# ShuoYangRobotics/Cerberus

Measured on NVIDIA H100. Metric: sliding-window solves/sec (10-frame x 150-feature windows), higher is better.
Workload: dtype f64

## Files before the change

### cerberus_b200/csrc/compat.h

```cpp
#pragma once
#include <math.h>
#include <stdint.h>
#if defined(CERB_CUSIM)
#include "cusim.h"
#else
#include <cuda_runtime.h>
#define CERB_HD __host__ __device__ __forceinline__
#define CERB_D __device__ __forceinline__
#define CERB_GLOBAL __global__
#define CERB_NOINLINE __device__ __noinline__
#define CERB_GRID_CONSTANT const __grid_constant__
#define CERB_DYN_SMEM(T, name)                                   \
    extern __shared__ __align__(16) unsigned char name##_raw[]; \
    T *name = reinterpret_cast<T *>(name##_raw)
#define CERB_LAUNCH(kernel, grid, block, smem, stream, ...) kernel<<<(grid), (block), (smem), (stream)>>>(__VA_ARGS__)
#define CERB_BAR_SYNC(id, nthreads) asm volatile("bar.sync %0, %1;" ::"r"(id), "r"(nthreads) : "memory")
#define CERB_CP_ASYNC8(dst_smem, src_global) asm volatile("cp.async.ca.shared.global [%0], [%1], 8;" ::"r"((unsigned)__cvta_generic_to_shared(dst_smem)), "l"(src_global) : "memory")
#define CERB_CP_ASYNC_WAIT() asm volatile("cp.async.commit_group;\n\tcp.async.wait_group 0;" ::: "memory")
#define CERB_SMEM_U32(p) ((unsigned)__cvta_generic_to_shared(p))
#define CERB_MBAR_INIT(bar) do { asm volatile("mbarrier.init.shared::cta.b64 [%0], 1;" ::"r"(CERB_SMEM_U32(bar))); asm volatile("fence.mbarrier_init.release.cluster;" ::: "memory"); } while (0)
#define CERB_BULK_G2S(dst_smem, src_global, bytes, bar) do {                                                                                        \
        asm volatile("fence.proxy.async.shared::cta;" ::: "memory");                                                                                 \
        asm volatile("mbarrier.arrive.expect_tx.shared::cta.b64 _, [%0], %1;" ::"r"(CERB_SMEM_U32(bar)), "r"((unsigned)(bytes)) : "memory");         \
        asm volatile("cp.async.bulk.shared::cluster.global.mbarrier::complete_tx::bytes [%0], [%1], %2, [%3];"                                      \
                     ::"r"(CERB_SMEM_U32(dst_smem)), "l"(src_global), "r"((unsigned)(bytes)), "r"(CERB_SMEM_U32(bar)) : "memory");                   \
    } while (0)
#define CERB_MBAR_WAIT(bar, parity) do {                                                                                                             \
        unsigned done_ = 0;                                                                                                                          \
        while (!done_) asm volatile("{ .reg .pred p; mbarrier.try_wait.parity.shared::cta.b64 p, [%1], %2; selp.u32 %0, 1, 0, p; }"                 \
                                    : "=r"(done_) : "r"(CERB_SMEM_U32(bar)), "r"((unsigned)(parity)) : "memory");                                    \
    } while (0)
#define CERB_ST_RELEASE_S32(p, v) asm volatile("st.release.cta.shared.s32 [%0], %1;" ::"r"(CERB_SMEM_U32(p)), "r"((int)(v)) : "memory")
#define CERB_LD_ACQUIRE_S32(p) ({ int v_; asm volatile("ld.acquire.cta.shared.s32 %0, [%1];" : "=r"(v_) : "r"(CERB_SMEM_U32(p)) : "memory"); v_; })
#define CERB_SPIN_PAUSE() __nanosleep(20)
#define CERB_BAR_ARRIVE(id, nthreads) asm volatile("bar.arrive %0, %1;" ::"r"(id), "r"(nthreads) : "memory")
#define CERB_DMMA(d0, d1, a, b, c0, c1) \
    asm volatile("mma.sync.aligned.m8n8k4.row.col.f64.f64.f64.f64 {%0,%1}, {%2}, {%3}, {%4,%5};" : "=d"(d0), "=d"(d1) : "d"(a), "d"(b), "d"(c0), "d"(c1))
#endif
```

### cerberus_b200/csrc/solve_kernel.cuh

```cuda
#pragma once
#include "eval_kernels.cuh"

namespace cerb {

#if defined(CERB_PHASE_TIMING) && !defined(CERB_CUSIM)
__device__ unsigned long long g_phase_cycles[48];
#define PH_DECL() long long ph_t = clock64()
#define PH_MARK_T(id, t) do { if ((threadIdx.x & 31) == 0) { const long long ph_n = clock64(); if (threadIdx.x == (t)) atomicAdd(&g_phase_cycles[id], (unsigned long long)(ph_n - ph_t)); ph_t = ph_n; } __syncwarp(); } while (0)
#define PH_MARK(id) PH_MARK_T(id, 0)
#define PH_ARG , long long &ph_t
#define PH_FWD , ph_t
#else
#define PH_DECL()
#define PH_MARK_T(id, t)
#define PH_MARK(id)
#define PH_ARG
#define PH_FWD
#endif

enum { CERB_WINDOW = 10, NX = 79, NYB = 13, NFR = 11, NY = 143, NR = 222, NRP = 224, HXX_SZ = 79 * 79, HXY_SZ = 79 * 143, X_TD = 78, SOLVE_THREADS = 256, FT = 64, TILE_LD = 33, NOBS_PLANES = 9 };
enum { HBLK = NYB * NYB, AD_SZ = NFR * HBLK, BO_SZ = (NFR - 1) * HBLK };
#ifndef CERB_SOLVE_MIN_BLOCKS
#define CERB_SOLVE_MIN_BLOCKS 1
#endif
// ... 263 lines not shown
            }
            double wjv[6] = {0, 0, 0, 0, 0, 0};
            double *t0 = T + tid, *t1 = T + 256 + tid;
            if (valid) {
                const d3 tic = ld3(x + ST_EX), tc = kind == PROJ_K1 ? tic : ld3(x + ST_EX + 7);
                const double *Rcp = kind == PROJ_K1 ? s.Rex : s.Rex + 9;
                const double tdv = x[ST_TD];
                const d3 pts_i = mk3(pix, piy, 1.0), vel_i = mk3(vix, viy, 0.0);
                const d3 pts_i_td = pts_i - (tdv - tdi) * vel_i;
                const double pjx_td = ov.px - (tdv - ov.td) * ov.vx, pjy_td = ov.py - (tdv - ov.td) * ov.vy;
                const double inv_l = lamf;
                const d3 p_ci = inv_l * pts_i_td;
                const d3 p_bi = mv33(ldm33(s.Rex), p_ci) + tic;
                d3 p_bj = p_bi;
                if (kind != PROJ_K3) p_bj = mTv33(ldm33(s.Rw + 9 * j), (mv33(ldm33(s.Rw + 9 * a), p_bi) + ld3(x + ST_POSE + 7 * a)) - ld3(x + ST_POSE + 7 * j));
                const d3 p_cj = mTv33(ldm33(Rcp), p_bj - tc);
                const double iz = 1.0 / p_cj.z;
                double r0 = P.sqrt_info * (p_cj.x * iz - pjx_td), r1 = P.sqrt_info * (p_cj.y * iz - pjy_td);
                double cf; const double hw = huber_weight(P.huber, r0 * r0 + r1 * r1, &cf);
                cost += cf;
                r0 *= hw; r1 *= hw;
                const double q = hw * P.sqrt_info * iz, c0 = -q * p_cj.x * iz, c1 = -q * p_cj.y * iz;
                const d3 e0 = mk3(q, 0.0, c0), e1 = mk3(0.0, q, c1);
#define VIS_U(M, u0, u1) const d3 u0 = mk3(q * (M)[0] + c0 * (M)[6], q * (M)[1] + c0 * (M)[7], q * (M)[2] + c0 * (M)[8]), u1 = mk3(q * (M)[3] + c1 * (M)[6], q * (M)[4] + c1 * (M)[7], q * (M)[5] + c1 * (M)[8])
#define VIS_PUT(col, a0, a1) do { t0[(col) * VT_LD] = (a0); t1[(col) * VT_LD] = (a1); } while (0)
#define VIS_PUT3(col, v0_, v1_) do { VIS_PUT(col, (v0_).x, (v1_).x); VIS_PUT((col) + 1, (v0_).y, (v1_).y); VIS_PUT((col) + 2, (v0_).z, (v1_).z); } while (0)
                const double *Tm = kind == PROJ_K3 ? s.lin + 540 : s.lin + 27 * (2 * (j - a - 1) + cam) + 18;
                VIS_U(Tm, uT0, uT1);
                const d3 ptl = kind == PROJ_K3 ? pts_i : pts_i_td;
                const double l0 = -inv_l * inv_l * dot3(uT0, ptl), l1 = -inv_l * inv_l * dot3(uT1, ptl);
                const double d0 = -inv_l * dot3(uT0, vel_i) + hw * P.sqrt_info * ov.vx, d1 = -inv_l * dot3(uT1, vel_i) + hw * P.sqrt_info * ov.vy;
                h += l0 * l0 + l1 * l1; gq += l0 * r0 + l1 * r1; wT += d0 * l0 + d1 * l1;
                VIS_PUT(6, d0, d1); VIS_PUT(7, r0, r1);
                const d3 uC0 = mk3(q * Rcp[0] + c0 * Rcp[2], q * Rcp[3] + c0 * Rcp[5], q * Rcp[6] + c0 * Rcp[8]);
                const d3 uC1 = mk3(q * Rcp[1] + c1 * Rcp[2], q * Rcp[4] + c1 * Rcp[5], q * Rcp[7] + c1 * Rcp[8]);
                const d3 er0 = cross3(e0, p_cj), er1 = cross3(e1, p_cj);
                const d3 et0 = cross3(p_ci, uT0), et1 = cross3(p_ci, uT1);
                d3 E0t0, E0t1, E0r0, E0r1, E1t0, E1t1, E1r0, E1r1;
                if (kind == PROJ_K3) {
                    for (int k = 0; k < 6; k++) { VIS_PUT(k, 0.0, 0.0); VIS_PUT(8 + k, 0.0, 0.0); }
                    E0t0 = uC0; E0t1 = uC1; E0r0 = et0; E0r1 = et1; E1t0 = -uC0; E1t1 = -uC1; E1r0 = er0; E1r1 = er1;
                } else {
                    const double *C = s.lin + 27 * (2 * (j - a - 1) + cam);
                    VIS_U(C, uA0, uA1);
                    VIS_U(C + 9, uR0, uR1);
                    const d3 ir0 = cross3(p_bi, uR0), ir1 = cross3(p_bi, uR1);
                    const d3 jr0 = cross3(uC0, p_bj), jr1 = cross3(uC1, p_bj);
                    VIS_PUT3(0, uA0, uA1); VIS_PUT3(3, ir0, ir1);
                    VIS_PUT3(8, -uA0, -uA1); VIS_PUT3(11, jr0, jr1);
                    wI[0] += uA0.x * l0 + uA1.x * l1; wI[1] += uA0.y * l0 + uA1.y * l1; wI[2] += uA0.z * l0 + uA1.z * l1;
                    wI[3] += ir0.x * l0 + ir1.x * l1; wI[4] += ir0.y * l0 + ir1.y * l1; wI[5] += ir0.z * l0 + ir1.z * l1;
                    wjv[0] = -(uA0.x * l0 + uA1.x * l1); wjv[1] = -(uA0.y * l0 + uA1.y * l1); wjv[2] = -(uA0.z * l0 + uA1.z * l1);
                    wjv[3] = jr0.x * l0 + jr1.x * l1; wjv[4] = jr0.y * l0 + jr1.y * l1; wjv[5] = jr0.z * l0 + jr1.z * l1;
                    if (kind == PROJ_K1) {
                        E0t0 = uR0 - uC0; E0t1 = uR1 - uC1; E0r0 = et0 + er0; E0r1 = et1 + er1;
                        E1t0 = mk3(0, 0, 0); E1t1 = E1t0; E1r0 = E1t0; E1r1 = E1t0;
                    } else {
                        E0t0 = uR0; E0t1 = uR1; E0r0 = et0; E0r1 = et1; E1t0 = -uC0; E1t1 = -uC1; E1r0 = er0; E1r1 = er1;
                    }
                }
                VIS_PUT3(14, E0t0, E0t1); VIS_PUT3(17, E0r0, E0r1); VIS_PUT3(20, E1t0, E1t1); VIS_PUT3(23, E1r0, E1r1);
                wE0[0] += E0t0.x * l0 + E0t1.x * l1; wE0[1] += E0t0.y * l0 + E0t1.y * l1; wE0[2] += E0t0.z * l0 + E0t1.z * l1;
                wE0[3] += E0r0.x * l0 + E0r1.x * l1; wE0[4] += E0r0.y * l0 + E0r1.y * l1; wE0[5] += E0r0.z * l0 + E0r1.z * l1;
                wE1[0] += E1t0.x * l0 + E1t1.x * l1; wE1[1] += E1t0.y * l0 + E1t1.y * l1; wE1[2] += E1t0.z * l0 + E1t1.z * l1;
                wE1[3] += E1r0.x * l0 + E1r1.x * l1; wE1[4] += E1r0.y * l0 + E1r1.y * l1; wE1[5] += E1r0.z * l0 + E1r1.z * l1;
#undef VIS_U
#undef VIS_PUT
#undef VIS_PUT3
            } else {
                for (int k = 0; k < VT_COLS; k++) { t0[k * VT_LD] = 0.0; t1[k * VT_LD] = 0.0; }
            }
            const bool wrow = valid && j != a;
            if (wrow && cam == 0) for (int k = 0; k < 6; k++) W[(size_t)(6 * j + k) * F + f] = wjv[k] * (prescale ? s.sc[6 * j + k] * slf : 1.0);
            __syncthreads();
            PH_MARK(21);
            double wprev[6] = {0, 0, 0, 0, 0, 0};
            if (wrow && cam == 1) for (int k = 0; k < 6; k++) wprev[k] = W[(size_t)(6 * j + k) * F + f];
            { const int jn = j + 2; ov.stereo = 0; if (ev && jn < a + nobs) obs_fetch(obs, stereo, mo, off + (jn - a), cam, ov); }
            {
                const int jw = j0 + (wid >> 2), hw = (wid >> 1) & 1, par = wid & 1;
                const bool k3 = (jw == a);
                const int nkt = (nc + 3) >> 2;
                const bool work = jw < NFR && par < nkt;
                double acc[10][2];
                for (int k = 0; k < 10; k++) { acc[k][0] = 0.0; acc[k][1] = 0.0; }
                if (work) {
                    const int rb0 = 256 * hw + 64 * (wid >> 2) + 4 * par;
                    if (!k3) {
                        double v0 = tq[0][rb0], v1 = tv[1] ? tq[1][rb0] : 0.0, v2 = tv[2] ? tq[2][rb0] : 0.0;
                        for (int ks = par; ks < nkt; ks += 2) {
                            const int rn = rb0 + 4 * (ks + 2 - par);
                            const bool more = ks + 2 < nkt;
                            const double n0 = more ? tq[0][rn] : 0.0, n1 = (more && tv[1]) ? tq[1][rn] : 0.0, n2 = (more && tv[2]) ? tq[2][rn] : 0.0;
                            CERB_DMMA(acc[0][0], acc[0][1], v0, v0, acc[0][0], acc[0][1]);
                            CERB_DMMA(acc[1][0], acc[1][1], v0, v1, acc[1][0], acc[1][1]);
                            CERB_DMMA(acc[2][0], acc[2][1], v0, v2, acc[2][0], acc[2][1]);
                            CERB_DMMA(acc[4][0], acc[4][1], v1, v1, acc[4][0], acc[4][1]);
                            CERB_DMMA(acc[5][0], acc[5][1], v1, v2, acc[5][0], acc[5][1]);
                            CERB_DMMA(acc[7][0], acc[7][1], v2, v2, acc[7][0], acc[7][1]);
                            v0 = n0; v1 = n1; v2 = n2;
                        }
                    }
                    {
                        const int rb1 = rb0 + 128;
                        double v0 = tq[0][rb1], v1 = (!k3 && tv[1]) ? tq[1][rb1] : 0.0, v2 = tv[2] ? tq[2][rb1] : 0.0, v3 = tv[3] ? tq[3][rb1] : 0.0;
                        for (int ks = par; ks < nkt; ks += 2) {
                            const int rn = rb1 + 4 * (ks + 2 - par);
                            const bool more = ks + 2 < nkt;
                            const double n0 = more ? tq[0][rn] : 0.0, n1 = (more && !k3 && tv[1]) ? tq[1][rn] : 0.0, n2 = (more && tv[2]) ? tq[2][rn] : 0.0, n3 = (more && tv[3]) ? tq[3][rn] : 0.0;
                            CERB_DMMA(acc[0][0], acc[0][1], v0, v0, acc[0][0], acc[0][1]);
                            CERB_DMMA(acc[2][0], acc[2][1], v0, v2, acc[2][0], acc[2][1]);
                            CERB_DMMA(acc[3][0], acc[3][1], v0, v3, acc[3][0], acc[3][1]);
                            CERB_DMMA(acc[7][0], acc[7][1], v2, v2, acc[7][0], acc[7][1]);
                            CERB_DMMA(acc[8][0], acc[8][1], v2, v3, acc[8][0], acc[8][1]);
                            CERB_DMMA(acc[9][0], acc[9][1], v3, v3, acc[9][0], acc[9][1]);
                            if (!k3) {
                                CERB_DMMA(acc[1][0], acc[1][1], v0, v1, acc[1][0], acc[1][1]);
                                CERB_DMMA(acc[4][0], acc[4][1], v1, v1, acc[4][0], acc[4][1]);
                                CERB_DMMA(acc[5][0], acc[5][1], v1, v2, acc[5][0], acc[5][1]);
                                CERB_DMMA(acc[6][0], acc[6][1], v1, v3, acc[6][0], acc[6][1]);
                            }
                            v0 = n0; v1 = n1; v2 = n2; v3 = n3;
                        }
                    }
                    PH_MARK(28);
                    const int o = (lane >> 2) * 8 + 2 * (lane & 3);
                    pp[0 * 64 + o] += acc[0][0]; pp[0 * 64 + o + 1] += acc[0][1];
                    pp[1 * 64 + o] += acc[2][0]; pp[1 * 64 + o + 1] += acc[2][1];
                    pp[2 * 64 + o] += acc[3][0]; pp[2 * 64 + o + 1] += acc[3][1];
                    pp[3 * 64 + o] += acc[7][0]; pp[3 * 64 + o + 1] += acc[7][1];
                    pp[4 * 64 + o] += acc[8][0]; pp[4 * 64 + o + 1] += acc[8][1];
                    pp[5 * 64 + o] += acc[9][0]; pp[5 * 64 + o + 1] += acc[9][1];
                }
                {
                    const int o = wid * VJ_SZ + (lane >> 2) * 8 + 2 * (lane & 3);
                    jp[o] = acc[1][0]; jp[o + 1] = acc[1][1];
                    jp[64 + o] = acc[4][0]; jp[64 + o + 1] = acc[4][1];
                    jp[128 + o] = acc[5][0]; jp[128 + o + 1] = acc[5][1];
                    jp[192 + o] = acc[6][0]; jp[192 + o + 1] = acc[6][1];
                }
            }
            if (wrow && cam == 1) for (int k = 0; k < 6; k++) W[(size_t)(6 * j + k) * F + f] = wprev[k] + wjv[k] * (prescale ? s.sc[6 * j + k] * slf : 1.0);
            PH_MARK(29);
            __syncthreads();
            PH_MARK(22);
            if (jbase >= 0) {
                _Pragma("unroll")
                for (int fj = 0; fj < 2; fj++) {
                    const int jf = j0 + fj;
                    if (jf >= NFR || jf == a) continue;
                    const double *q = jp + (4 * fj) * VJ_SZ + tid;
                    smem_base[jbase + jca * a + jcj * jf] += ((q[0] + q[VJ_SZ]) + q[2 * VJ_SZ]) + q[3 * VJ_SZ];
                }
            }
            PH_MARK(23);
        }
        __syncthreads();
        {
            double *ex = T;
            ex[0 * 256 + tid] = h; ex[1 * 256 + tid] = gq; ex[2 * 256 + tid] = wT;
            for (int k = 0; k < 6; k++) { ex[(3 + k) * 256 + tid] = wI[k]; ex[(9 + k) * 256 + tid] = wE0[k]; ex[(15 + k) * 256 + tid] = wE1[k]; }
        }
        __syncthreads();
        for (int e = tid; e < VP_SZ; e += SOLVE_THREADS) {
            double v = 0.0;
            for (int wq = 0; wq < 8; wq++) v += ((wq < 5) ? s.Ju + 8 * VJ_SZ + VP_SZ * wq : s.tile + VT_SZ + VP_SZ * (wq - 5))[e];
            const int blk = e >> 6, ra = (e >> 3) & 7, rb = e & 7;
            const int ga = blk < 3 ? 0 : (blk < 5 ? 2 : 3), gb = blk == 0 ? 0 : (blk == 1 || blk == 3 ? 2 : 3);
            vis_scatter(s, ga, gb, ra, rb, a, a, v);
        }
        if (tid < 64 && ev) {
            const double *ex = T;
            double q[21];
            for (int k = 0; k < 21; k++) q[k] = ((ex[k * 256 + tid] + ex[k * 256 + 64 + tid]) + ex[k * 256 + 128 + tid]) + ex[k * 256 + 192 + tid];
            hh[f] = q[0] * slf * slf; gl[f] = q[1] * slf;
            W[(size_t)X_TD * F + f] = q[2] * (prescale ? s.sc[X_TD] * slf : 1.0);
            for (int k = 0; k < 6; k++) {
                W[(size_t)(6 * a + k) * F + f] = q[3 + k] * (prescale ? s.sc[6 * a + k] * slf : 1.0);
                W[(size_t)(66 + k) * F + f] = q[9 + k] * (prescale ? s.sc[66 + k] * slf : 1.0);
                W[(size_t)(72 + k) * F + f] = q[15 + k] * (prescale ? s.sc[72 + k] * slf : 1.0);
            }
        }
        __syncthreads();
        PH_MARK(24);
    }
    return cost;
}

CERB_D void imu_lin_all(const SolveParams &P, Smem &s, int w, const double *x, bool want_jac, int tid) {
    if (tid < CERB_WINDOW) {
        const double *pre = P.pre + ((size_t)w * CERB_WINDOW + tid) * PRE_STRIDE;
        IMULegLin *L = reinterpret_cast<IMULegLin *>(s.lin + 96 * tid);
        imu_leg_linearize(pre, x + ST_POSE + 7 * tid, x + ST_SB + 9 * tid, x + ST_LB + 4 * tid, x + ST_POSE + 7 * (tid + 1),
                          x + ST_SB + 9 * (tid + 1), x + ST_LB + 4 * (tid + 1), P.G, want_jac, L);
    }
    __syncthreads();
}

CERB_D double prior_residual(const SolveParams &P, Smem &s, int w, const double *x, int tid) {
    const int *meta = P.prior_meta + (size_t)w * PRIOR_META_STRIDE;
    if (!meta[0]) return 0.0;
    const int n = meta[1], nb = meta[2];
    const double *J = P.prior_J + (size_t)w * PRIOR_LD * PRIOR_LD, *r0 = P.prior_r + (size_t)w * PRIOR_LD, *x0 = P.prior_x0 + (size_t)w * 16 * 9;
    if (tid < nb) {
        const int kind = meta[4 + 3 * tid], index = meta[5 + 3 * tid], col = meta[6 + 3 * tid];
        prior_block_dx(kind, x + prior_block_state_offset(kind, index), x0 + 9 * tid, s.pdx + col);
    }
    __syncthreads();
    int parts = SOLVE_THREADS / n; if (parts > 4) parts = 4; if (parts < 1) parts = 1;
    const int kc = (n + parts - 1) / parts;
    double *part = s.red;
    for (int e = tid; e < parts * n; e += SOLVE_THREADS) {
        const int p = e / n, i = e % n;
        const int k1 = (p + 1) * kc < n ? (p + 1) * kc : n;
        double t = 0.0;
        for (int k = p * kc; k < k1; k++) t += J[(size_t)k * n + i] * s.pdx[k];
        part[p * PRIOR_LD + i] = t;
    }
    __syncthreads();
    double cost = 0.0;
    for (int i = tid; i < n; i += SOLVE_THREADS) {
        double t = r0[i];
// ... 194 lines not shown
    for (int k = tid; k < NR; k += SOLVE_THREADS) s.g[k] += gp[k];
    __syncthreads();
    PH_MARK(27);
    return cost;
}

CERB_D void apply_plus(const Smem &s, const double *delta, const double *lam, const double *dlam, double *lamc, int nF, bool ex_open, bool td_open, int tid) {
    if (tid < 11) pose_plus(s.xs + ST_POSE + 7 * tid, delta + 6 * tid, s.xc + ST_POSE + 7 * tid);
    else if (tid < 13) {
        const int e = tid - 11;
        if (ex_open) pose_plus(s.xs + ST_EX + 7 * e, delta + 66 + 6 * e, s.xc + ST_EX + 7 * e);
        else for (int k = 0; k < 7; k++) s.xc[ST_EX + 7 * e + k] = s.xs[ST_EX + 7 * e + k];
    }
    for (int k = tid; k < 99; k += SOLVE_THREADS) { const int f = k / 9, c = k % 9; s.xc[ST_SB + k] = s.xs[ST_SB + k] + delta[NX + NYB * f + c]; }
    for (int k = tid; k < 44; k += SOLVE_THREADS) { const int f = k / 4, c = k % 4; s.xc[ST_LB + k] = s.xs[ST_LB + k] + delta[NX + NYB * f + 9 + c]; }
    if (tid == 0) s.xc[ST_TD] = td_open ? s.xs[ST_TD] + delta[X_TD] : s.xs[ST_TD];
    for (int f = tid; f < nF; f += SOLVE_THREADS) lamc[f] = lam[f] + dlam[f];
    __syncthreads();
}

CERB_D double ambient_sq(const double *a, const double *b, const double *la, const double *lb, int nF, bool ex_open, bool lb_open, bool td_open, int tid) {
    double t = 0.0;
    for (int k = tid; k < ST_SIZE; k += SOLVE_THREADS) {
        if (k >= ST_LB && k < ST_EX && !lb_open) continue;
        if (k >= ST_EX && k < ST_TD && !ex_open) continue;
        if (k == ST_TD && !td_open) continue;
        const double v = b ? a[k] - b[k] : a[k];
        t += v * v;
    }
    for (int f = tid; f < nF; f += SOLVE_THREADS) { const double v = lb ? la[f] - lb[f] : la[f]; t += v * v; }
    return t;
}

template <int W> struct TTPlan;
#define CERB_TT_PLAN(W, NR_, NB_, ...) template <> struct TTPlan<W> { static constexpr int nr = NR_, nb = NB_; static CERB_HD int tab(int i) { constexpr int t[] = {__VA_ARGS__}; return t[i]; } };
CERB_TT_PLAN(0, 4, 7, 0, 1, 2, 3, 0, 0, 0,   0, 0, 1, 0, 1, 0, 1,   0, 1, 1, 2, 2, 3, 3)
CERB_TT_PLAN(1, 4, 7, 2, 3, 4, 5, 0, 0, 0,   0, 0, 1, 0, 1, 0, 1,   0, 1, 1, 2, 2, 3, 3)
CERB_TT_PLAN(2, 4, 7, 4, 5, 6, 7, 0, 0, 0,   0, 0, 1, 0, 1, 0, 1,   0, 1, 1, 2, 2, 3, 3)
CERB_TT_PLAN(3, 4, 7, 6, 7, 8, 9, 0, 0, 0,   0, 0, 1, 0, 1, 0, 1,   0, 1, 1, 2, 2, 3, 3)
CERB_TT_PLAN(4, 6, 7, 8, 9, 0, 1, 4, 5, 0,   0, 0, 1, 2, 3, 2, 3,   0, 1, 1, 4, 4, 5, 5)
CERB_TT_PLAN(5, 6, 7, 0, 1, 6, 7, 8, 9, 0,   0, 0, 0, 0, 1, 1, 1,   2, 3, 4, 5, 2, 3, 4)
CERB_TT_PLAN(6, 7, 7, 1, 9, 2, 6, 7, 8, 3,   0, 2, 2, 2, 2, 6, 6,   1, 3, 4, 5, 1, 3, 4)
CERB_TT_PLAN(7, 5, 6, 3, 4, 5, 8, 9, 0, 0,   0, 0, 1, 1, 2, 2, 0,   3, 4, 3, 4, 3, 4, 0)
template <int W> CERB_D void ttt_warp(Smem &s, int lane) {
    typedef TTPlan<W> PL;
    const double *pr[7];
    _Pragma("unroll")
    for (int u = 0; u < 7; u++) {
        const int r = 8 * PL::tab(u < PL::nr ? u : 0) + (lane >> 2);
        pr[u] = (r < NX ? s.Hxy + r * NY : s.yv + NX) + (lane & 3);
    }
    double acc[7][2], fv[7];
    _Pragma("unroll")
    for (int k = 0; k < 7; k++) { acc[k][0] = 0.0; acc[k][1] = 0.0; }
    _Pragma("unroll")
    for (int u = 0; u < 7; u++) fv[u] = (u < PL::nr) ? pr[u][0] : 0.0;
    for (int q0 = 0; q0 < NY; q0 += 4) {
        const int qn = q0 + 4;
        const bool take = qn < NY && qn + (lane & 3) < NY;
        double fn[7];
        _Pragma("unroll")
        for (int u = 0; u < 7; u++) fn[u] = (u < PL::nr && take) ? pr[u][qn] : 0.0;
        _Pragma("unroll")
        for (int k = 0; k < 7; k++) if (k < PL::nb) CERB_DMMA(acc[k][0], acc[k][1], fv[PL::tab(7 + k)], fv[PL::tab(14 + k)], acc[k][0], acc[k][1]);
        _Pragma("unroll")
        for (int u = 0; u < 7; u++) fv[u] = fn[u];
    }
    _Pragma("unroll")
    for (int k = 0; k < 7; k++) {
        if (k >= PL::nb) continue;
        const int ba = PL::tab(PL::tab(7 + k)), bb = PL::tab(PL::tab(14 + k));
        const int a = 8 * ba + (lane >> 2);
        for (int e = 0; e < 2; e++) {
            const int b = 8 * bb + 2 * (lane & 3) + e;
            if (a > b || a >= NX || b > NX) continue;
            if (b == NX) s.yv[a] -= acc[k][e];
            else s.Hxx[b * NX + a] -= acc[k][e];
        }
    }
}

template <int W> struct SCPlan;
#define CERB_SC_PLAN(W, NR_, NB_, ...) template <> struct SCPlan<W> { static constexpr int nr = NR_, nb = NB_; static CERB_HD int tab(int i) { constexpr int t[] = {__VA_ARGS__}; return t[i]; } };
CERB_SC_PLAN(0, 8, 8, 0, 1, 2, 3, 4, 5, 6, 7, 0,   0, 0, 0, 0, 0, 0, 0, 0,   0, 1, 2, 3, 4, 5, 6, 7)
CERB_SC_PLAN(1, 9, 8, 0, 8, 9, 1, 2, 3, 4, 5, 6,   0, 0, 3, 3, 3, 3, 3, 3,   1, 2, 3, 4, 5, 6, 7, 8)
CERB_SC_PLAN(2, 9, 8, 1, 7, 8, 9, 2, 3, 4, 5, 6,   0, 0, 0, 4, 4, 4, 4, 4,   1, 2, 3, 4, 5, 6, 7, 8)
CERB_SC_PLAN(3, 8, 8, 2, 7, 8, 9, 3, 4, 5, 6, 0,   0, 0, 0, 4, 4, 4, 4, 4,   1, 2, 3, 4, 5, 6, 7, 1)
CERB_SC_PLAN(4, 7, 8, 3, 8, 9, 4, 5, 6, 7, 0, 0,   0, 0, 3, 3, 3, 3, 3, 3,   1, 2, 3, 4, 5, 6, 1, 2)
CERB_SC_PLAN(5, 5, 8, 5, 6, 7, 8, 9, 0, 0, 0, 0,   0, 0, 0, 0, 0, 1, 1, 1,   0, 1, 2, 3, 4, 1, 2, 3)
CERB_SC_PLAN(6, 4, 7, 6, 7, 8, 9, 0, 0, 0, 0, 0,   0, 1, 1, 1, 2, 2, 3, 0,   3, 1, 2, 3, 2, 3, 3, 0)
enum { SC_LDW = 36 };
template <int W> CERB_D void schur_tile(const double *tw, double (&acc)[8][2], int lane) {
    typedef SCPlan<W> PL;
    const double *pr[9];
    _Pragma("unroll")
    for (int u = 0; u < 9; u++) pr[u] = tw + (8 * PL::tab(u < PL::nr ? u : 0) + (lane >> 2)) * SC_LDW + (lane & 3);
    double fv[9];
    _Pragma("unroll")
    for (int u = 0; u < 9; u++) fv[u] = (u < PL::nr) ? pr[u][0] : 0.0;
    _Pragma("unroll")
    for (int ks = 0; ks < 8; ks++) {
        double fn[9];
        _Pragma("unroll")
        for (int u = 0; u < 9; u++) fn[u] = (u < PL::nr && ks < 7) ? pr[u][4 * (ks + 1)] : 0.0;
        _Pragma("unroll")
        for (int k = 0; k < 8; k++) if (k < PL::nb) CERB_DMMA(acc[k][0], acc[k][1], fv[PL::tab(9 + k)], fv[PL::tab(17 + k)], acc[k][0], acc[k][1]);
        _Pragma("unroll")
        for (int u = 0; u < 9; u++) fv[u] = fn[u];
    }
}
template <int W> CERB_D void schur_scatter(Smem &s, const double (&acc)[8][2], int lane) {
    typedef SCPlan<W> PL;
    _Pragma("unroll")
    for (int k = 0; k < 8; k++) {
        if (k >= PL::nb) continue;
        const int a = 8 * PL::tab(PL::tab(9 + k)) + (lane >> 2);
        for (int e = 0; e < 2; e++) {
            const int b = 8 * PL::tab(PL::tab(17 + k)) + 2 * (lane & 3) + e;
            if (a > b || a >= NX || b > NX) continue;
            if (b == NX) s.yv[a] -= acc[k][e];
            else { s.Hxx[b * NX + a] -= acc[k][e]; if (a != b) s.Hxx[a * NX + b] -= acc[k][e]; }
        }
    }
}

CERB_D bool build_prior_image(const SolveParams &P, Smem &s, int w, double *pimg, int tid) {
    const int *pmeta = P.prior_meta + (size_t)w * PRIOR_META_STRIDE;
    const bool has_prior = pmeta[0] != 0;
    if (has_prior) {
        const int n = pmeta[1], nb = pmeta[2];
        for (int k = tid; k < PIMG_SZ; k += SOLVE_THREADS) pimg[k] = 0.0;
        if (tid < nb) {
            const int kind = pmeta[4 + 3 * tid], index = pmeta[5 + 3 * tid], col = pmeta[6 + 3 * tid];
            const int local = (kind == 0 || kind == 3) ? 6 : prior_block_size(kind);
            for (int k = 0; k < local; k++) {
                int d;
                if (kind == 0) d = 6 * index + k;
                else if (kind == 3) d = 66 + 6 * index + k;
                else if (kind == 1) d = -(1 + NYB * index + k);
                else if (kind == 2) d = -(1 + NYB * index + 9 + k);
                else d = X_TD;
                s.ti[TI_PRIOR_MAP + col + k] = d;
            }
        }
        __syncthreads();
        Smem si = s; si.Hxx = pimg; si.Hxy = pimg + PIMG_HXY; si.Ad = pimg + PIMG_HXY + HXY_SZ; si.Bo = pimg + PIMG_HXY + HXY_SZ + AD_SZ;
        const double *Hp = P.prior_Hp + (size_t)w * PRIOR_LD * PRIOR_LD;
        for (int idx = tid; idx < n * n; idx += SOLVE_THREADS) {
            const int a = idx / n, b = idx % n;
            if (b < a) continue;
            scatter_H(si, s.ti[TI_PRIOR_MAP + a], s.ti[TI_PRIOR_MAP + b], Hp[a * PRIOR_LD + b]);
        }
    }
    return has_prior;
}

CERB_D void build_imu_plan(const Smem &s, const double *smem_base, int *plan, int tid) {
    if (tid >= 32) return;
    int q = 0;
    for (int mi = 0; mi < 5; mi++)
        for (int ni = mi; ni < 5; ni++, q++)
            for (int e = 0; e < 2; e++) {
                const int la = 8 * mi + (tid >> 2), lb = 8 * ni + 2 * (tid & 3) + e;
                int px = (int)(s.idg - smem_base) + tid, py = 256 << 12;
                if (la <= lb && lb <= 38 && la != 38) {
                    double *p0[2], *p1[2];
                    for (int i = 0; i < 2; i++) {
                        const int da = imu_col_dest(i, la);
                        if (lb == 38) { p0[i] = da >= 0 ? s.g + da : s.g + NX + (-da - 1); p1[i] = nullptr; }
                        else scatter_addr(s, da, imu_col_dest(i, lb), &p0[i], &p1[i]);
                    }
                    px = (int)(p0[0] - smem_base);
                    py = (int)(p0[1] - p0[0]) | (((p1[0] ? (int)(p1[0] - p0[0]) : 0) + 256) << 12);
                }
                plan[(2 * (q * 2 + e)) * 32 + tid] = px; plan[(2 * (q * 2 + e) + 1) * 32 + tid] = py;
            }
}
CERB_D void build_chunks(const int *fstart, Smem &s, int *chunks, int n_end) {
    int n = 0, c0 = 0;
    while (c0 < n_end) {
        chunks[1 + n] = c0;
        const int a = fstart[c0];
        int e = c0 + 1;
        while (e < n_end && e < c0 + 64 && fstart[e] == a) e++;
        if (n < TI_CACHED_CHUNKS) { s.ti[TI_CHUNK_CACHE + 2 * n] = c0; s.ti[TI_CHUNK_CACHE + 2 * n + 1] = ((e - c0) << 8) | a; }
        n++; c0 = e;
    }
    chunks[1 + n] = n_end; chunks[0] = n; s.ti[TI_NCHUNKS] = n;
}
struct Win { int w, nF; bool ex_open, lb_open, td_open, has_prior, bulk_ok; double *lam; CtaWs ws; };
struct PriorCopy { unsigned par0, par1; bool hxx_prefetched; };
CERB_D void linearize(const SolveParams &P, Smem &s, const Win &c, PriorCopy &pc, const double *xl, const double *laml, bool first, int tid PH_ARG) {
    const int F = c.ws.F, nF = c.nF;
    double *sca = s.sca, *W = c.ws.W, *hh = c.ws.hh, *gl = c.ws.gl, *sl = c.ws.sl, *pimg = c.ws.pimg;
    if (!c.has_prior) { for (int k = tid; k < HXX_SZ; k += SOLVE_THREADS) s.Hxx[k] = 0.0; }
    else if (c.bulk_ok) {
        if (!pc.hxx_prefetched) { __syncthreads(); if (tid == 0) CERB_BULK_G2S(s.Hxx, pimg, PIMG_HXY * 8, &s.mbar[0]); }
        CERB_MBAR_WAIT(&s.mbar[0], pc.par0); pc.par0 ^= 1;
    } else { if (!pc.hxx_prefetched) copy_g2s_async(s.Hxx, pimg, HXX_SZ, tid); CERB_CP_ASYNC_WAIT(); }
    pc.hxx_prefetched = false;
    for (int k = tid; k < NRP; k += SOLVE_THREADS) s.g[k] = 0.0;
    load_geometry(xl, s, tid);
    double part[2];
    PH_MARK(0);
// ... 58 lines not shown
    if (tid == 0) {
        if (iteration >= P.max_iters) { sca[S_DONE] = 1; sca[S_TERM] = 1; }
        else if (sca[S_GMAX] <= P.gtol) { sca[S_DONE] = 1; sca[S_TERM] = 0; }
        else if (sca[S_RADIUS] <= P.min_radius) { sca[S_DONE] = 1; sca[S_TERM] = 0; }
        else if (!(sca[S_XCOST] == sca[S_XCOST]) || fabs(sca[S_XCOST]) > 1e300) { sca[S_DONE] = 1; sca[S_TERM] = 2; }
    }
    __syncthreads();
    return sca[S_DONE] != 0.0;
}
CERB_D void dogleg_diagonal(Smem &s, const Win &c, int tid PH_ARG) {
    const int nF = c.nF;
    double *sca = s.sca, *Dl = c.ws.Dl, *ghl = c.ws.ghl, *stl = c.ws.stl;
    for (int k = tid; k < NR; k += SOLVE_THREADS) {
        const double d = (k < NX) ? s.Hxx[k * NX + k] : s.Ad[((k - NX) / NYB) * HBLK + ((k - NX) % NYB) * (NYB + 1)];
        const double D = sqrt(fmin(fmax(d, 1e-6), 1e32));
        s.D[k] = D; s.gh[k] = s.g[k] / D; s.stp[k] = s.gh[k] / D;
    }
    for (int f = tid; f < nF; f += SOLVE_THREADS) { const double D = sqrt(fmin(fmax(c.ws.hh[f], 1e-6), 1e32)); Dl[f] = D; ghl[f] = c.ws.gl[f] / D; stl[f] = ghl[f] / D; }
    __syncthreads();
    double part[2] = {0.0, 0.0};
    for (int k = tid; k < AD_SZ; k += SOLVE_THREADS) { const int f = k / HBLK, a = (k % HBLK) / NYB, b = k % NYB; part[0] += s.stp[NX + NYB * f + a] * s.Ad[k] * s.stp[NX + NYB * f + b]; }
    for (int k = tid; k < BO_SZ; k += SOLVE_THREADS) { const int f = k / HBLK, a = (k % HBLK) / NYB, b = k % NYB; part[0] += 2.0 * s.stp[NX + NYB * f + a] * s.Bo[k] * s.stp[NX + NYB * (f + 1) + b]; }
    for (int f = tid; f < nF; f += SOLVE_THREADS) part[1] += ghl[f] * ghl[f];
    for (int k = tid; k < NR; k += SOLVE_THREADS) part[1] += s.gh[k] * s.gh[k];
    double tot[2];
    block_sum<2>(part, s.red, tot, tid);
    if (tid == 0) { sca[S_GNORM2] = tot[1]; sca[S_VHV] = tot[0]; sca[S_OK] = 1; }
    PH_MARK(4);
}
CERB_D void chain_cholesky(Smem &s, int *chain_done, int lane PH_ARG) {
    const bool act = lane < NYB;
    const int r = act ? lane : 0;
    double m[NYB];
    _Pragma("unroll")
    for (int c = 0; c < NYB; c++) m[c] = 0.0;
    _Pragma("unroll 1")
    for (int f = 0; f < NFR; f++) {
        double *A = s.Ad + f * HBLK;
        double a[NYB], invd[NYB], myinv = 1.0;
        _Pragma("unroll")
        for (int c = 0; c < NYB; c++) a[c] = A[r * NYB + c];
        if (f > 0) {
            const double *Mp = s.Bo + (f - 1) * HBLK;
            _Pragma("unroll")
            for (int c = 0; c < NYB; c++) { double t = 0.0; _Pragma("unroll") for (int q = 0; q < NYB; q++) t += m[q] * Mp[c * NYB + q]; a[c] -= t; }
        }
        _Pragma("unroll")
        for (int j = 0; j < NYB; j++) {
            double d = __shfl_sync(0xffffffffu, a[j], j);
            if (!(d > 0.0)) { if (lane == 0) s.sca[S_OK] = 0; d = 1.0; }
            const double inv = rsqrt(d);
            invd[j] = inv;
            if (lane == j) myinv = inv;
            const double l = (lane == j) ? d * inv : a[j] * inv;
            a[j] = l;
            double *colb = s.chain_col + 16 * (j & 1);
            if (act) colb[lane] = l;
            __syncwarp();
            _Pragma("unroll")
            for (int k = j + 1; k < NYB; k++) a[k] -= l * colb[k];
        }
        if (act) { _Pragma("unroll") for (int c = 0; c < NYB; c++) if (c <= r) A[r * NYB + c] = a[c]; s.idg[NYB * f + r] = myinv; }
        __syncwarp();
        if (f < NFR - 1) {
            double *B = s.Bo + f * HBLK;
            double t[NYB];
            _Pragma("unroll")
            for (int c = 0; c < NYB; c++) t[c] = B[c * NYB + r];
            _Pragma("unroll")
            for (int c = 0; c < NYB; c++) {
                m[c] = t[c] * invd[c];
                _Pragma("unroll")
                for (int c2 = c + 1; c2 < NYB; c2++) t[c2] -= m[c] * A[c2 * NYB + c];
            }
            __syncwarp();
            if (act) { _Pragma("unroll") for (int c = 0; c < NYB; c++) B[r * NYB + c] = m[c]; }
            __syncwarp();
        }
        __threadfence_block(); __syncwarp();
        if (lane == 0) CERB_ST_RELEASE_S32(chain_done, f + 1);
    }
    PH_MARK(6);
}
CERB_D void schur_tile_w(int wq, const double *tw, double (&acc)[8][2], int lane) {
    switch (wq) { case 0: schur_tile<0>(tw, acc, lane); break; case 1: schur_tile<1>(tw, acc, lane); break; case 2: schur_tile<2>(tw, acc, lane); break;
                  case 3: schur_tile<3>(tw, acc, lane); break; case 4: schur_tile<4>(tw, acc, lane); break; case 5: schur_tile<5>(tw, acc, lane); break;
                  default: schur_tile<6>(tw, acc, lane); break; }
}
CERB_D void schur_scatter_w(int wq, Smem &s, const double (&acc)[8][2], int lane) {
    switch (wq) { case 0: schur_scatter<0>(s, acc, lane); break; case 1: schur_scatter<1>(s, acc, lane); break; case 2: schur_scatter<2>(s, acc, lane); break;
                  case 3: schur_scatter<3>(s, acc, lane); break; case 4: schur_scatter<4>(s, acc, lane); break; case 5: schur_scatter<5>(s, acc, lane); break;
                  default: schur_scatter<6>(s, acc, lane); break; }
}
CERB_D void ttt_warp_w(int wq, Smem &s, int lane) {
    switch (wq) { case 0: ttt_warp<0>(s, lane); break; case 1: ttt_warp<1>(s, lane); break; case 2: ttt_warp<2>(s, lane); break; case 3: ttt_warp<3>(s, lane); break;
                  case 4: ttt_warp<4>(s, lane); break; case 5: ttt_warp<5>(s, lane); break; case 6: ttt_warp<6>(s, lane); break; default: ttt_warp<7>(s, lane); break; }
}
CERB_D void lambda_schur(Smem &s, const Win &c, double mu, int tid PH_ARG) {
    const int F = c.ws.F, nF = c.nF;
    const double *W = c.ws.W, *hh = c.ws.hh, *gl = c.ws.gl, *Dl = c.ws.Dl, *stl = c.ws.stl;
    const int t2 = tid - 32, n2 = SOLVE_THREADS - 32;
    const int wq = (tid >> 5) - 1, lane = tid & 31;
    const int LDW = SC_LDW;
    double *tw = s.Ju;
    double *sinv = nF <= 1024 ? s.wj : c.ws.sinv;
    {
        const double *v = s.stp;
        double pv = 0.0;
        for (int k = t2; k < NX * NX; k += n2) pv += v[k / NX] * s.Hxx[k] * v[k % NX];
        for (int k = t2; k < NX * NY; k += n2) pv += 2.0 * v[k / NY] * s.Hxy[k] * v[NX + k % NY];
        for (int f = t2; f < nF; f += n2) {
            double wv = 0.0;
            for (int a = 0; a < NX; a++) wv += W[(size_t)a * F + f] * v[a];
            pv += 2.0 * stl[f] * wv + hh[f] * stl[f] * stl[f];
        }
        for (int o = 16; o > 0; o >>= 1) pv += __shfl_sync(0xffffffffu, pv, (lane + o) & 31);
        if (lane == 0) s.lin[wq] = pv;
        CERB_BAR_SYNC(1, n2);
        for (int k = t2; k < NX; k += n2) s.Hxx[k * NX + k] += mu * s.D[k] * s.D[k];
    }
    PH_MARK_T(19, 32);
    for (int f = t2; f < nF; f += n2) sinv[f] = rsqrt(hh[f] + mu * Dl[f] * Dl[f]);
    double acc[8][2];
    _Pragma("unroll")
    for (int k = 0; k < 8; k++) { acc[k][0] = 0.0; acc[k][1] = 0.0; }
    CERB_BAR_SYNC(1, n2);
    double buf[12];
    auto fetch = [&](int f0) {
        const int nf = (nF - f0) < 32 ? (nF - f0) : 32;
        _Pragma("unroll")
        for (int u = 0; u < 12; u++) {
            const int e = t2 + u * n2, a = e >> 5, f = e & 31;
            buf[u] = (e < 80 * 32 && f < nf) ? (a < NX ? W[(size_t)a * F + f0 + f] : (a == NX ? gl[f0 + f] : 0.0)) : 0.0;
        }
    };
    fetch(0);
    PH_MARK_T(37, 32);
    for (int f0 = 0; f0 < nF; f0 += 32) {
        const int nf = (nF - f0) < 32 ? (nF - f0) : 32;
        _Pragma("unroll")
        for (int u = 0; u < 12; u++) {
            const int e = t2 + u * n2, a = e >> 5, f = e & 31;
            if (e < 80 * 32) tw[a * LDW + f] = (f < nf) ? buf[u] * sinv[f0 + f] : 0.0;
        }
        CERB_BAR_SYNC(1, n2);
        PH_MARK_T(38, 32);
        if (f0 + 32 < nF) fetch(f0 + 32);
        schur_tile_w(wq, tw, acc, lane);
        CERB_BAR_SYNC(1, n2);
        PH_MARK_T(39, 32);
    }
    schur_scatter_w(wq, s, acc, lane);
    PH_MARK_T(7, 32);
}
CERB_D void forward_subst(Smem &s, const int *chain_done, int t2) {
    if (t2 <= NX) {
        double *row = (t2 < NX) ? s.Hxy + t2 * NY : s.yv + NX;
        double tp[NYB];
        _Pragma("unroll")
        for (int k = 0; k < NYB; k++) tp[k] = 0.0;
        _Pragma("unroll 1")
        for (int f = 0; f < NFR; f++) {
            while (CERB_LD_ACQUIRE_S32(chain_done) <= f) { CERB_SPIN_PAUSE(); }
            __threadfence_block();
            const double *L = s.Ad + f * HBLK, *idg = s.idg + NYB * f;
            double *t = row + NYB * f;
            double tc[NYB];
            _Pragma("unroll")
            for (int r = 0; r < NYB; r++) tc[r] = t[r];
            if (f > 0) {
                const double *M = s.Bo + (f - 1) * HBLK;
                _Pragma("unroll")
                for (int r = 0; r < NYB; r++) { double acc = 0.0; _Pragma("unroll") for (int q = 0; q < NYB; q++) acc += M[r * NYB + q] * tp[q]; tc[r] -= acc; }
            }
            _Pragma("unroll")
            for (int c = 0; c < NYB; c++) {
                tc[c] *= idg[c];
                _Pragma("unroll")
                for (int r = c + 1; r < NYB; r++) tc[r] -= L[r * NYB + c] * tc[c];
            }
            _Pragma("unroll")
            for (int r = 0; r < NYB; r++) { t[r] = tc[r]; tp[r] = tc[r]; }
        }
    }
}
CERB_D void panel_cholesky(Smem &s, int tid) {
    const int wq = tid >> 5, lane = tid & 31;
    auto factor_diag = [&](int c0, int nb, double *Lkk) {
        const bool act = lane < nb;
        const int r = act ? lane : 0;
        double a[8];
        _Pragma("unroll")
        for (int c = 0; c < 8; c++) a[c] = (c < nb && c <= r) ? s.Hxx[(c0 + r) * NX + c0 + c] : 0.0;
        double myinv = 1.0;
        _Pragma("unroll")
        for (int j = 0; j < 8; j++) {
            double d = __shfl_sync(0xffffffffu, a[j], j);
            if (j < nb && !(d > 0.0)) { if (lane == 0) s.sca[S_OK] = 0; }
            if (!(d > 0.0)) d = 1.0;
            const double inv = rsqrt(d);
            if (lane == j) myinv = inv;
            const double l = (lane == j) ? d * inv : a[j] * inv;
            a[j] = l;
            _Pragma("unroll")
            for (int k = j + 1; k < 8; k++) { const double lk = __shfl_sync(0xffffffffu, l, k); a[k] -= l * lk; }
        }
        if (act) {
            _Pragma("unroll")
// ... 483 lines not shown
```

Measured before the change: 29250.

## Pair FP64 8x8x4 DMMAs into m16n8k4 instructions in visibility and Schur tiles

Replaces pairs of m8n8k4 FP64 mma.sync ops sharing a B operand with single m16n8k4 instructions, in both the visibility-block accumulation and the Schur complement tile kernel. The Schur tiling plan tables are rewritten so each warp issues fewer, larger MMAs, and the scatter is updated for the new accumulator layout, including transposed indexing for some blocks. This cuts MMA instruction count and issue overhead. It also redistributes work across warps and relies on index mapping that is easy to get wrong.

```diff
diff --git a/cerberus_b200/csrc/compat.h b/cerberus_b200/csrc/compat.h
--- a/cerberus_b200/csrc/compat.h
+++ b/cerberus_b200/csrc/compat.h
@@ -3,6 +3,7 @@
 #include <stdint.h>
 #if defined(CERB_CUSIM)
 #include "cusim.h"
+#define CERB_DMMA_16x8x4(d0, d1, d2, d3, a0, a1, b) do { CERB_DMMA(d0, d1, a0, b, d0, d1); CERB_DMMA(d2, d3, a1, b, d2, d3); } while (0)
 #else
 #include <cuda_runtime.h>
 #define CERB_HD __host__ __device__ __forceinline__
@@ -36,4 +37,7 @@
 #define CERB_BAR_ARRIVE(id, nthreads) asm volatile("bar.arrive %0, %1;" ::"r"(id), "r"(nthreads) : "memory")
 #define CERB_DMMA(d0, d1, a, b, c0, c1) \
     asm volatile("mma.sync.aligned.m8n8k4.row.col.f64.f64.f64.f64 {%0,%1}, {%2}, {%3}, {%4,%5};" : "=d"(d0), "=d"(d1) : "d"(a), "d"(b), "d"(c0), "d"(c1))
+#define CERB_DMMA_16x8x4(d0, d1, d2, d3, a0, a1, b)                                                                                   \
+    asm volatile("mma.sync.aligned.m16n8k4.row.col.f64.f64.f64.f64 {%0,%1,%2,%3}, {%4,%5}, {%6}, {%0,%1,%2,%3};"                    \
+                 : "+d"(d0), "+d"(d1), "+d"(d2), "+d"(d3) : "d"(a0), "d"(a1), "d"(b))
 #endif
diff --git a/cerberus_b200/csrc/solve_kernel.cuh b/cerberus_b200/csrc/solve_kernel.cuh
--- a/cerberus_b200/csrc/solve_kernel.cuh
+++ b/cerberus_b200/csrc/solve_kernel.cuh
@@ -369,8 +369,9 @@
                 const bool k3 = (jw == a);
                 const int nkt = (nc + 3) >> 2;
                 const bool work = jw < NFR && par < nkt;
-                double acc[10][2];
-                for (int k = 0; k < 10; k++) { acc[k][0] = 0.0; acc[k][1] = 0.0; }
+                double acc[5][4];
+                for (int k = 0; k < 5; k++) { acc[k][0] = 0.0; acc[k][1] = 0.0; acc[k][2] = 0.0; acc[k][3] = 0.0; }
+#define VIS_Q(q, ga, gb, gc) CERB_DMMA_16x8x4(acc[q][0], acc[q][1], acc[q][2], acc[q][3], ga, gb, gc)
                 if (work) {
                     const int rb0 = 256 * hw + 64 * (wid >> 2) + 4 * par;
                     if (!k3) {
@@ -379,12 +380,7 @@
                             const int rn = rb0 + 4 * (ks + 2 - par);
                             const bool more = ks + 2 < nkt;
                             const double n0 = more ? tq[0][rn] : 0.0, n1 = (more && tv[1]) ? tq[1][rn] : 0.0, n2 = (more && tv[2]) ? tq[2][rn] : 0.0;
-                            CERB_DMMA(acc[0][0], acc[0][1], v0, v0, acc[0][0], acc[0][1]);
-                            CERB_DMMA(acc[1][0], acc[1][1], v0, v1, acc[1][0], acc[1][1]);
-                            CERB_DMMA(acc[2][0], acc[2][1], v0, v2, acc[2][0], acc[2][1]);
-                            CERB_DMMA(acc[4][0], acc[4][1], v1, v1, acc[4][0], acc[4][1]);
-                            CERB_DMMA(acc[5][0], acc[5][1], v1, v2, acc[5][0], acc[5][1]);
-                            CERB_DMMA(acc[7][0], acc[7][1], v2, v2, acc[7][0], acc[7][1]);
+                            VIS_Q(0, v0, v2, v0); VIS_Q(1, v1, v0, v1); VIS_Q(2, v2, v1, v2);
                             v0 = n0; v1 = n1; v2 = n2;
                         }
                     }
@@ -395,36 +391,27 @@
                             const int rn = rb1 + 4 * (ks + 2 - par);
                             const bool more = ks + 2 < nkt;
                             const double n0 = more ? tq[0][rn] : 0.0, n1 = (more && !k3 && tv[1]) ? tq[1][rn] : 0.0, n2 = (more && tv[2]) ? tq[2][rn] : 0.0, n3 = (more && tv[3]) ? tq[3][rn] : 0.0;
-                            CERB_DMMA(acc[0][0], acc[0][1], v0, v0, acc[0][0], acc[0][1]);
-                            CERB_DMMA(acc[2][0], acc[2][1], v0, v2, acc[2][0], acc[2][1]);
-                            CERB_DMMA(acc[3][0], acc[3][1], v0, v3, acc[3][0], acc[3][1]);
-                            CERB_DMMA(acc[7][0], acc[7][1], v2, v2, acc[7][0], acc[7][1]);
-                            CERB_DMMA(acc[8][0], acc[8][1], v2, v3, acc[8][0], acc[8][1]);
-                            CERB_DMMA(acc[9][0], acc[9][1], v3, v3, acc[9][0], acc[9][1]);
-                            if (!k3) {
-                                CERB_DMMA(acc[1][0], acc[1][1], v0, v1, acc[1][0], acc[1][1]);
-                                CERB_DMMA(acc[4][0], acc[4][1], v1, v1, acc[4][0], acc[4][1]);
-                                CERB_DMMA(acc[5][0], acc[5][1], v1, v2, acc[5][0], acc[5][1]);
-                                CERB_DMMA(acc[6][0], acc[6][1], v1, v3, acc[6][0], acc[6][1]);
-                            }
+                            VIS_Q(0, v0, v2, v0); VIS_Q(2, v2, v1, v2); VIS_Q(3, v0, v2, v3); VIS_Q(4, v3, v1, v3);
+                            if (!k3) VIS_Q(1, v1, v0, v1);
                             v0 = n0; v1 = n1; v2 = n2; v3 = n3;
                         }
                     }
                     PH_MARK(28);
-                    const int o = (lane >> 2) * 8 + 2 * (lane & 3);
+                    const int o = (lane >> 2) * 8 + 2 * (lane & 3), ot = 2 * (lane & 3) * 8 + (lane >> 2);
                     pp[0 * 64 + o] += acc[0][0]; pp[0 * 64 + o + 1] += acc[0][1];
-                    pp[1 * 64 + o] += acc[2][0]; pp[1 * 64 + o + 1] += acc[2][1];
+                    pp[1 * 64 + ot] += acc[0][2]; pp[1 * 64 + ot + 8] += acc[0][3];
                     pp[2 * 64 + o] += acc[3][0]; pp[2 * 64 + o + 1] += acc[3][1];
-                    pp[3 * 64 + o] += acc[7][0]; pp[3 * 64 + o + 1] += acc[7][1];
-                    pp[4 * 64 + o] += acc[8][0]; pp[4 * 64 + o + 1] += acc[8][1];
-                    pp[5 * 64 + o] += acc[9][0]; pp[5 * 64 + o + 1] += acc[9][1];
+                    pp[3 * 64 + o] += acc[2][0]; pp[3 * 64 + o + 1] += acc[2][1];
+                    pp[4 * 64 + o] += acc[3][2]; pp[4 * 64 + o + 1] += acc[3][3];
+                    pp[5 * 64 + o] += acc[4][0]; pp[5 * 64 + o + 1] += acc[4][1];
                 }
+#undef VIS_Q
                 {
                     const int o = wid * VJ_SZ + (lane >> 2) * 8 + 2 * (lane & 3);
-                    jp[o] = acc[1][0]; jp[o + 1] = acc[1][1];
-                    jp[64 + o] = acc[4][0]; jp[64 + o + 1] = acc[4][1];
-                    jp[128 + o] = acc[5][0]; jp[128 + o + 1] = acc[5][1];
-                    jp[192 + o] = acc[6][0]; jp[192 + o + 1] = acc[6][1];
+                    jp[o] = acc[1][2]; jp[o + 1] = acc[1][3];
+                    jp[64 + o] = acc[1][0]; jp[64 + o + 1] = acc[1][1];
+                    jp[128 + o] = acc[2][2]; jp[128 + o + 1] = acc[2][3];
+                    jp[192 + o] = acc[4][2]; jp[192 + o + 1] = acc[4][3];
                 }
             }
             if (wrow && cam == 1) for (int k = 0; k < 6; k++) W[(size_t)(6 * j + k) * F + f] = wprev[k] + wjv[k] * (prescale ? s.sc[6 * j + k] * slf : 1.0);
@@ -785,15 +772,15 @@
 
 template <int W> struct SCPlan;
 #define CERB_SC_PLAN(W, NR_, NB_, ...) template <> struct SCPlan<W> { static constexpr int nr = NR_, nb = NB_; static CERB_HD int tab(int i) { constexpr int t[] = {__VA_ARGS__}; return t[i]; } };
-CERB_SC_PLAN(0, 8, 8, 0, 1, 2, 3, 4, 5, 6, 7, 0,   0, 0, 0, 0, 0, 0, 0, 0,   0, 1, 2, 3, 4, 5, 6, 7)
-CERB_SC_PLAN(1, 9, 8, 0, 8, 9, 1, 2, 3, 4, 5, 6,   0, 0, 3, 3, 3, 3, 3, 3,   1, 2, 3, 4, 5, 6, 7, 8)
-CERB_SC_PLAN(2, 9, 8, 1, 7, 8, 9, 2, 3, 4, 5, 6,   0, 0, 0, 4, 4, 4, 4, 4,   1, 2, 3, 4, 5, 6, 7, 8)
-CERB_SC_PLAN(3, 8, 8, 2, 7, 8, 9, 3, 4, 5, 6, 0,   0, 0, 0, 4, 4, 4, 4, 4,   1, 2, 3, 4, 5, 6, 7, 1)
-CERB_SC_PLAN(4, 7, 8, 3, 8, 9, 4, 5, 6, 7, 0, 0,   0, 0, 3, 3, 3, 3, 3, 3,   1, 2, 3, 4, 5, 6, 1, 2)
-CERB_SC_PLAN(5, 5, 8, 5, 6, 7, 8, 9, 0, 0, 0, 0,   0, 0, 0, 0, 0, 1, 1, 1,   0, 1, 2, 3, 4, 1, 2, 3)
-CERB_SC_PLAN(6, 4, 7, 6, 7, 8, 9, 0, 0, 0, 0, 0,   0, 1, 1, 1, 2, 2, 3, 0,   3, 1, 2, 3, 2, 3, 3, 0)
+CERB_SC_PLAN(0, 9, 4, 0, 1, 2, 3, 4, 5, 6, 7, 9,   0, 2, 4, 6, 0,   1, 3, 5, 7, -1,   8, 8, 8, 8, 0)
+CERB_SC_PLAN(1, 9, 4, 0, 1, 2, 3, 4, 5, 6, 7, 8,   0, 2, 4, 6, 0,   1, 3, 5, 7, -1,   8, 8, 8, 8, 0)
+CERB_SC_PLAN(2, 8, 5, 0, 1, 2, 3, 4, 5, 6, 7, 0,   0, 2, 4, 6, 0,   1, 3, 5, 7, 1,    7, 7, 7, 7, 1)
+CERB_SC_PLAN(3, 2, 2, 8, 9, 0, 0, 0, 0, 0, 0, 0,   0, 0, 0, 0, 0,   1, -1, -1, -1, -1, 1, 0, 0, 0, 0)
+CERB_SC_PLAN(4, 6, 5, 0, 1, 2, 3, 4, 5, 0, 0, 0,   0, 2, 4, 0, 2,   1, 3, 5, 1, 3,    5, 5, 5, 3, 3)
+CERB_SC_PLAN(5, 5, 5, 0, 1, 2, 3, 4, 0, 0, 0, 0,   0, 2, 4, 0, 2,   1, 3, -1, 1, -1,  4, 4, 4, 2, 2)
+CERB_SC_PLAN(6, 7, 5, 0, 1, 2, 3, 4, 5, 6, 0, 0,   0, 2, 4, 6, 0,   1, 3, 5, -1, -1,  6, 6, 6, 6, 0)
 enum { SC_LDW = 36 };
-template <int W> CERB_D void schur_tile(const double *tw, double (&acc)[8][2], int lane) {
+template <int W> CERB_D void schur_tile(const double *tw, double (&acc)[5][4], int lane) {
     typedef SCPlan<W> PL;
     const double *pr[9];
     _Pragma("unroll")
@@ -807,22 +794,27 @@
         _Pragma("unroll")
         for (int u = 0; u < 9; u++) fn[u] = (u < PL::nr && ks < 7) ? pr[u][4 * (ks + 1)] : 0.0;
         _Pragma("unroll")
-        for (int k = 0; k < 8; k++) if (k < PL::nb) CERB_DMMA(acc[k][0], acc[k][1], fv[PL::tab(9 + k)], fv[PL::tab(17 + k)], acc[k][0], acc[k][1]);
+        for (int k = 0; k < 5; k++)
+            if (k < PL::nb) CERB_DMMA_16x8x4(acc[k][0], acc[k][1], acc[k][2], acc[k][3], fv[PL::tab(9 + k)], PL::tab(14 + k) >= 0 ? fv[PL::tab(14 + k) < 0 ? 0 : PL::tab(14 + k)] : 0.0, fv[PL::tab(19 + k)]);
         _Pragma("unroll")
         for (int u = 0; u < 9; u++) fv[u] = fn[u];
     }
 }
-template <int W> CERB_D void schur_scatter(Smem &s, const double (&acc)[8][2], int lane) {
+template <int W> CERB_D void schur_scatter(Smem &s, const double (&acc)[5][4], int lane) {
     typedef SCPlan<W> PL;
     _Pragma("unroll")
-    for (int k = 0; k < 8; k++) {
+    for (int k = 0; k < 5; k++) {
         if (k >= PL::nb) continue;
-        const int a = 8 * PL::tab(PL::tab(9 + k)) + (lane >> 2);
-        for (int e = 0; e < 2; e++) {
-            const int b = 8 * PL::tab(PL::tab(17 + k)) + 2 * (lane & 3) + e;
-            if (a > b || a >= NX || b > NX) continue;
-            if (b == NX) s.yv[a] -= acc[k][e];
-            else { s.Hxx[b * NX + a] -= acc[k][e]; if (a != b) s.Hxx[a * NX + b] -= acc[k][e]; }
+        _Pragma("unroll")
+        for (int h = 0; h < 2; h++) {
+            if (h == 1 && PL::tab(14 + k) < 0) continue;
+            const int a = 8 * PL::tab(PL::tab(h ? 14 + k : 9 + k)) + (lane >> 2);
+            for (int e = 0; e < 2; e++) {
+                const int b = 8 * PL::tab(PL::tab(19 + k)) + 2 * (lane & 3) + e;
+                if (a > b || a >= NX || b > NX) continue;
+                if (b == NX) s.yv[a] -= acc[k][2 * h + e];
+                else { s.Hxx[b * NX + a] -= acc[k][2 * h + e]; if (a != b) s.Hxx[a * NX + b] -= acc[k][2 * h + e]; }
+            }
         }
     }
 }
@@ -1047,12 +1039,12 @@
     }
     PH_MARK(6);
 }
-CERB_D void schur_tile_w(int wq, const double *tw, double (&acc)[8][2], int lane) {
+CERB_D void schur_tile_w(int wq, const double *tw, double (&acc)[5][4], int lane) {
     switch (wq) { case 0: schur_tile<0>(tw, acc, lane); break; case 1: schur_tile<1>(tw, acc, lane); break; case 2: schur_tile<2>(tw, acc, lane); break;
                   case 3: schur_tile<3>(tw, acc, lane); break; case 4: schur_tile<4>(tw, acc, lane); break; case 5: schur_tile<5>(tw, acc, lane); break;
                   default: schur_tile<6>(tw, acc, lane); break; }
 }
-CERB_D void schur_scatter_w(int wq, Smem &s, const double (&acc)[8][2], int lane) {
+CERB_D void schur_scatter_w(int wq, Smem &s, const double (&acc)[5][4], int lane) {
     switch (wq) { case 0: schur_scatter<0>(s, acc, lane); break; case 1: schur_scatter<1>(s, acc, lane); break; case 2: schur_scatter<2>(s, acc, lane); break;
                   case 3: schur_scatter<3>(s, acc, lane); break; case 4: schur_scatter<4>(s, acc, lane); break; case 5: schur_scatter<5>(s, acc, lane); break;
                   default: schur_scatter<6>(s, acc, lane); break; }
@@ -1086,9 +1078,9 @@
     }
     PH_MARK_T(19, 32);
     for (int f = t2; f < nF; f += n2) sinv[f] = rsqrt(hh[f] + mu * Dl[f] * Dl[f]);
-    double acc[8][2];
+    double acc[5][4];
     _Pragma("unroll")
-    for (int k = 0; k < 8; k++) { acc[k][0] = 0.0; acc[k][1] = 0.0; }
+    for (int k = 0; k < 5; k++) { acc[k][0] = 0.0; acc[k][1] = 0.0; acc[k][2] = 0.0; acc[k][3] = 0.0; }
     CERB_BAR_SYNC(1, n2);
     double buf[12];
     auto fetch = [&](int f0) {
```

Measured after the change: 29950 (median of 6 runs). 1.02x the previous value.
